# charlie-foxtrot/RTLSDR-Airband

Measured on AMD Instinct MI355X. Metric: IQ Msamples/sec channelized+demodulated per node; % HBM roofline, higher is better.
Workload: dtype i8x3->i32->f32 (stage 1), f32 (stage 2)

## Files before the change

### include/airband_hip.h

```cpp
#ifndef AIRBAND_HIP_H
#define AIRBAND_HIP_H

#include <stddef.h>
#include <stdint.h>

#ifdef __cplusplus
extern "C" {
#endif

#define AIRBAND_HIP_ABI_VERSION 2u

#define AIRBAND_HIP_OK 0
#define AIRBAND_HIP_ENODEV (-1)
#define AIRBAND_HIP_EBADSIZE (-2)
#define AIRBAND_HIP_ENOMEM (-3)
#define AIRBAND_HIP_EINVAL (-4)
#define AIRBAND_HIP_EAGAIN (-5)
#define AIRBAND_HIP_ERUNTIME (-6)

#define AIRBAND_SFMT_U8 1
#define AIRBAND_SFMT_S8 2
#define AIRBAND_SFMT_S16 3
#define AIRBAND_SFMT_F32 4

// ... 160 lines not shown
int airband_hip_collect_active(airband_hip_handle* h, int64_t* n_active, int32_t* channel_index, float* waveout, float* iq_out, char* axc_all);

int airband_hip_device_active(airband_hip_handle* h, int32_t** d_index, int32_t** d_count, float** d_rows, float** d_iq_rows);

int airband_hip_stream_wait_results(airband_hip_handle* h, void* stream);

int airband_hip_flush(airband_hip_handle* h);

int airband_hip_synchronize(airband_hip_handle* h);


int airband_hip_process_bins(airband_hip_handle* h, const float* wavein, const float* iq_in);

int airband_hip_read_bins(airband_hip_handle* h, float* wavein, float* iq_in);
int airband_hip_read_bins_channels(airband_hip_handle* h, int64_t first_channel, int64_t n_channels, float* wavein, float* iq_in);

int airband_hip_read_trace(airband_hip_handle* h, uint8_t* state);
int airband_hip_read_trace_channels(airband_hip_handle* h, int64_t first_channel, int64_t n_channels, uint8_t* state);

int airband_hip_channel_constants(const airband_hip_handle* h, int32_t channel_index, double* out_vals);

int airband_hip_derive_constants(const airband_hip_config* cfg, int32_t channel_index, double* out_vals);

int airband_hip_dft_selftest(const airband_hip_config* cfg, int32_t windows, double* max_rel_err);

int airband_hip_last_timings(airband_hip_handle* h, float* ms4);

int airband_hip_timing_totals(airband_hip_handle* h, double* ms4_sum, int64_t* n_batches, int32_t reset);

const char* airband_hip_build_info(void);

int airband_hip_regrouped(const airband_hip_handle* h);

const char* airband_hip_channelizer_name(const airband_hip_handle* h);

const char* airband_hip_channelizer_reason(const airband_hip_handle* h);

int64_t airband_hip_wide_hop_lds_bytes(int32_t fft_size, int32_t hop_bytes, int32_t sample_format);

int airband_hip_set_signal_plan(airband_hip_handle* h, const int64_t* carriers, int32_t n_carriers, int32_t noise_q8, const int16_t* sin_table4096);

int airband_hip_set_signal_plan_shift(airband_hip_handle* h, int32_t n_plans, uint32_t shift_step);

int airband_hip_generate_iq(airband_hip_handle* h, void* d_iq, size_t stride_bytes, uint64_t start_byte, size_t nbytes, uint64_t seed,
                            int32_t device_index_offset, void* stream);

#ifdef __cplusplus
}
#endif
#endif
```

### rtlsdr-airband_amd/__init__.py

```python
from __future__ import annotations

import ctypes as C
import importlib
import os
from typing import Optional, Sequence

import numpy as np

capi = importlib.import_module(__name__ + ".capi")
siggen = importlib.import_module(__name__ + ".siggen")
_build = importlib.import_module(__name__ + "._build")

HERE = os.path.dirname(os.path.abspath(__file__))
LIB_PATH = os.environ.get("AIRBAND_HIP_LIB") or os.path.join(HERE, "libairband_hip.so")

EXPORTS = [
    "airband_hip_prepare", "airband_hip_set_mixers", "airband_hip_release", "airband_hip_get_geometry", "airband_hip_last_error", "airband_hip_submit",
    "airband_hip_process", "airband_hip_process_device", "airband_hip_collect", "airband_hip_collect_mixers", "airband_hip_device_results",
    "airband_hip_synchronize", "airband_hip_process_bins", "airband_hip_read_bins", "airband_hip_read_trace", "airband_hip_channel_constants",
    "airband_hip_derive_constants", "airband_hip_last_timings", "airband_hip_channelizer_name", "airband_hip_set_signal_plan", "airband_hip_generate_iq",
    "airband_hip_flush", "airband_hip_timing_totals", "airband_hip_stream_wait_results", "airband_hip_mixer_enable_input",
    "airband_hip_device_enable", "airband_hip_gpu_count", "airband_hip_build_info", "airband_hip_dft_selftest", "airband_hip_collect_channels", "airband_hip_read_bins_channels", "airband_hip_read_trace_channels",
    "airband_hip_batch_ready", "airband_hip_mixer_set_stereo", "airband_hip_comm_unique_id", "airband_hip_comm_init_rank", "airband_hip_comm_init_all",
    "airband_hip_comm_group_begin", "airband_hip_comm_group_end", "airband_hip_allreduce_mixers", "airband_hip_add_mixers", "airband_hip_comm_destroy", "airband_hip_clear_mixers", "airband_hip_set_signal_plan_shift", "airband_hip_regrouped",
    "airband_hip_prepare_scan", "airband_hip_set_freq_index", "airband_hip_freq_stats",
    "airband_hip_set_output_gate", "airband_hip_collect_active", "airband_hip_device_active",
    "airband_hip_channelizer_reason", "airband_hip_wide_hop_lds_bytes",
]

_lib = None


class DevicePtr:

    def __init__(self, ptr: int, shape, typestr: str):
        self.__cuda_array_interface__ = dict(shape=tuple(shape), typestr=typestr, data=(int(ptr), False), version=2)


class AirbandError(RuntimeError):
    def __init__(self, code: int, text: str):
        super().__init__("airband_hip error %d: %s" % (code, text))
        self.code = code


def load_library() -> C.CDLL:
    global _lib
    if _lib is not None:
        return _lib
    if not os.path.exists(LIB_PATH):
        raise RuntimeError("libairband_hip.so is missing: run __graft_entry__.build() / python rtlsdr-airband_amd/_build.py (no CPU fallback exists)")
    try:
        import torch
    except Exception:
        pass
    L = C.CDLL(LIB_PATH)
    vp, i32, i64, u64, sz = C.c_void_p, C.c_int32, C.c_int64, C.c_uint64, C.c_size_t
    L.airband_hip_prepare.argtypes = [C.POINTER(capi.Config), C.POINTER(vp)]
    L.airband_hip_prepare_scan.argtypes = [C.POINTER(capi.Config), C.POINTER(capi.ScanCfg), i32, C.POINTER(vp)]
    L.airband_hip_set_freq_index.argtypes = [vp, i32, i32]
    L.airband_hip_freq_stats.argtypes = [vp, i32, i32, C.POINTER(capi.ChannelStats)]
# ... 14 lines not shown
    L.airband_hip_allreduce_mixers.argtypes = [vp, vp]
    L.airband_hip_add_mixers.argtypes = [vp, vp]
    L.airband_hip_comm_destroy.argtypes = [vp]
    L.airband_hip_clear_mixers.argtypes = [vp]
    L.airband_hip_comm_group_begin.argtypes = []
    L.airband_hip_comm_group_end.argtypes = []
    L.airband_hip_process_device.argtypes = [vp, vp, sz, vp]
    L.airband_hip_collect.argtypes = [vp, vp, vp, vp, vp]
    L.airband_hip_collect_channels.argtypes = [vp, i64, i64, vp, vp, vp, vp]
    L.airband_hip_read_bins_channels.argtypes = [vp, i64, i64, vp, vp]
    L.airband_hip_read_trace_channels.argtypes = [vp, i64, i64, vp]
    L.airband_hip_set_output_gate.argtypes = [vp, vp, i64]
    L.airband_hip_collect_active.argtypes = [vp, C.POINTER(i64), vp, vp, vp, vp]
    L.airband_hip_device_active.argtypes = [vp] + [C.POINTER(vp)] * 4
    L.airband_hip_collect_mixers.argtypes = [vp, vp, vp, vp]
    L.airband_hip_device_results.argtypes = [vp] + [C.POINTER(vp)] * 6
    L.airband_hip_synchronize.argtypes = [vp]
    L.airband_hip_process_bins.argtypes = [vp, vp, vp]
    L.airband_hip_read_bins.argtypes = [vp, vp, vp]
    L.airband_hip_read_trace.argtypes = [vp, vp]
    L.airband_hip_channel_constants.argtypes = [vp, i32, C.POINTER(C.c_double)]
    L.airband_hip_derive_constants.argtypes = [C.POINTER(capi.Config), i32, C.POINTER(C.c_double)]
    L.airband_hip_last_timings.argtypes = [vp, C.POINTER(C.c_float)]
    L.airband_hip_channelizer_name.argtypes = [vp]
    L.airband_hip_channelizer_name.restype = C.c_char_p
    L.airband_hip_channelizer_reason.argtypes = [vp]
    L.airband_hip_channelizer_reason.restype = C.c_char_p
    L.airband_hip_wide_hop_lds_bytes.argtypes = [i32, i32, i32]
    L.airband_hip_wide_hop_lds_bytes.restype = i64
    L.airband_hip_set_signal_plan.argtypes = [vp, vp, i32, i32, vp]
    L.airband_hip_generate_iq.argtypes = [vp, vp, sz, u64, sz, u64, i32, vp]
    L.airband_hip_set_signal_plan_shift.argtypes = [vp, i32, C.c_uint32]
    L.airband_hip_regrouped.argtypes = [vp]
    L.airband_hip_dft_selftest.argtypes = [C.POINTER(capi.Config), i32, C.POINTER(C.c_double)]
    L.airband_hip_build_info.argtypes = []
    L.airband_hip_build_info.restype = C.c_char_p
    L.airband_hip_flush.argtypes = [vp]
    L.airband_hip_mixer_enable_input.argtypes = [vp, i32, i32]
    L.airband_hip_device_enable.argtypes = [vp, i32, i32]
    L.airband_hip_gpu_count.argtypes = []
    L.airband_hip_stream_wait_results.argtypes = [vp, vp]
    L.airband_hip_timing_totals.argtypes = [vp, C.POINTER(C.c_double), C.POINTER(C.c_int64), i32]
    _lib = L
    return L


def make_config(devices: Sequence[dict], *, wave_rate: int, fft_log: int = 9, fm_demod: int = 0, flags: int = 0, hip_device: int = 0):
    keep, devs = [], []
    for dev in devices:
        dc, arr = capi.device_cfg(**dev)
        keep.append(arr)
        devs.append(dc)
    darr = (capi.DeviceCfg * len(devs))(*devs)
    keep.append(darr)
    cfg = capi.Config(capi.ABI_VERSION, flags, fft_log, wave_rate, fm_demod, hip_device, len(devs), C.cast(darr, C.POINTER(capi.DeviceCfg)))
    return cfg, keep


def derive_constants(devices: Sequence[dict], channel_index: int, *, wave_rate: int, fft_log: int = 9, fm_demod: int = 0):
    L = load_library()
    cfg, keep = make_config(devices, wave_rate=wave_rate, fft_log=fft_log, fm_demod=fm_demod)
    v = (C.c_double * 16)()
    rc = L.airband_hip_derive_constants(C.byref(cfg), channel_index, v)
    if rc != 0:
        raise AirbandError(rc, (L.airband_hip_last_error(None) or b"").decode())
    return list(v)
# ... 173 lines not shown
        w = np.empty((n, B), np.float32)
        q = np.empty((n, 2 * B), np.float32)
        self._check(self.L.airband_hip_read_bins_channels(self.h, int(first_channel), n, w.ctypes.data, q.ctypes.data))
        return w, q

    def read_trace(self, first_channel: int = 0, n_channels: Optional[int] = None) -> np.ndarray:
        n = self.total_channels - first_channel if n_channels is None else int(n_channels)
        t = np.empty((n, self.B), np.uint8)
        self._check(self.L.airband_hip_read_trace_channels(self.h, int(first_channel), n, t.ctypes.data))
        return t

    def constants(self, channel_index: int):
        v = (C.c_double * 16)()
        self._check(self.L.airband_hip_channel_constants(self.h, channel_index, v))
        return list(v)

    def last_timings(self):
        v = (C.c_float * 4)()
        self._check(self.L.airband_hip_last_timings(self.h, v))
        return dict(channelizer_ms=v[0], demod_ms=v[1], emit_ms=v[2], batch_ms=v[3])

    def timing_totals(self, reset: bool = False):
        v = (C.c_double * 4)()
        n = C.c_int64(0)
        self._check(self.L.airband_hip_timing_totals(self.h, v, C.byref(n), 1 if reset else 0))
        return dict(channelizer_ms=v[0], demod_ms=v[1], emit_ms=v[2], batch_ms=v[3], batches=int(n.value))

    def channelizer_name(self) -> str:
        return self.L.airband_hip_channelizer_name(self.h).decode()

    def channelizer_reason(self) -> str:
        return (self.L.airband_hip_channelizer_reason(self.h) or b"").decode()

    def build_info(self) -> str:
        return self.L.airband_hip_build_info().decode()

    def set_mixers(self, n_mixers: int, inputs: Sequence[tuple]):
        arr = (capi.MixerInput * len(inputs))(*[capi.MixerInput(int(a), int(b), int(c), float(d), float(e)) for a, b, c, d, e in inputs])
        self._check(self.L.airband_hip_set_mixers(self.h, n_mixers, arr, len(inputs)))
        self.n_mixers = n_mixers

    def mixer_enable_input(self, input_index: int, enabled: bool):
        self._check(self.L.airband_hip_mixer_enable_input(self.h, input_index, 1 if enabled else 0))

    def mixer_set_stereo(self, mixer: int, stereo: bool):
        self._check(self.L.airband_hip_mixer_set_stereo(self.h, int(mixer), 1 if stereo else 0))

    @staticmethod
    def comm_unique_id() -> bytes:
        buf = (C.c_uint8 * 128)()
        rc = load_library().airband_hip_comm_unique_id(buf)
        if rc < 0:
            raise AirbandError(rc, (load_library().airband_hip_last_error(None) or b"").decode())
        return bytes(buf)

    def comm_init_rank(self, unique_id: bytes, nranks: int, rank: int):
        assert len(unique_id) == 128
        self._check(self.L.airband_hip_comm_init_rank(self.h, (C.c_uint8 * 128).from_buffer_copy(unique_id), int(nranks), int(rank)))

    def allreduce_mixers(self, stream: int = 0):
        self._check(self.L.airband_hip_allreduce_mixers(self.h, C.c_void_p(stream)))

    def add_mixers(self, src: "AirbandHip"):
        self._check(self.L.airband_hip_add_mixers(self.h, src.h))

    def clear_mixers(self):
# ... 63 lines not shown
```

### rtlsdr-airband_amd/csrc/airband_hip.cpp

```cpp
#include <hip/hip_runtime.h>
#include <dlfcn.h>

#include <atomic>
#include <cstdio>
#include <cstdlib>
#include <cstring>
#include <memory>
#include <mutex>
#include <string>
#include <vector>

#include "handle.h"
#include "kernels.h"
#include "scan_bank.h"

#ifndef AB_PRIVATE_TABLE_BUDGET
#define AB_PRIVATE_TABLE_BUDGET ((size_t)8 << 30)
#endif

#ifndef AB_F32_TABLE_BUDGET
#define AB_F32_TABLE_BUDGET ((size_t)512 << 20)
#endif

using namespace airband;
// ... 79 lines not shown
        h->evp_state[i] = 0;
    }
    h->evp_state[i] |= (uint8_t)(1u << half);
    return h->evp[i];
}

void launch_retune_tables(airband_hip_handle* h, hipStream_t s, int epoch) {
    RetuneArgs ra;
    ra.cc = h->d_cc.p;
    ra.cs = h->d_cs.p;
    ra.dev = h->d_dev.p;
    ra.ext_to_slot = h->d_ext_to_slot.p;
    ra.item_dev = h->d_item_dev.p;
    ra.item_group = h->d_item_group.p;
    ra.item_bset = h->d_item_bset.p;
    ra.item_private = h->d_item_private.p;
    ra.item_home = h->d_item_home.p;
    ra.bset_bin = h->d_bset_bin.p;
    ra.bfrag = h->d_bfrag.p;
    ra.corr = h->d_bcorr.p;
    ra.ftab = h->use_f32 ? h->d_ftab.p : nullptr;
    ra.window = h->d_window.p;
    ra.n_items = (int)h->plan.item_dev.size();
    ra.fft_size = h->plan.fft_size;
    ra.n_shared = h->plan.n_shared_bsets;
    ra.moved_epoch = h->d_bset_bin.p + (size_t)h->plan.n_bsets * 8;
    ra.epoch = epoch;
    launch_retune(ra, s);
}

struct FrontRows {
    int first_row, n_hops;
};

FrontRows front_rows(const airband_hip_handle* h) {
    const bool first = h->front_batches == 0;
    return {first ? 0 : AB_AGC_EXTRA, first ? h->B + AB_AGC_EXTRA : h->B};
}

template <class Args>
void fill_front_args(Args& a, const airband_hip_handle* h, const void* d_iq, size_t stride_bytes, int row0, FrontRows r) {
    a.iq = (const uint8_t*)d_iq;
    a.iq_stride = (long)stride_bytes;
    a.dev = h->d_dev.p;
    a.cc = h->d_cc.p;
    a.ext_to_slot = h->d_ext_to_slot.p;
    a.mag = h->d_mag.p;
    a.iq_bins = h->d_iq.p;
    a.row0 = row0;
    a.ring_rows = h->R;
    a.first_row = r.first_row;
    a.n_hops = r.n_hops;
}

ChannelizerArgs fft_args(const airband_hip_handle* h, const void* d_iq, size_t stride_bytes, int row0, FrontRows r, int spectrum_only) {
    const Plan& p = h->plan;
    ChannelizerArgs ca;
    fill_front_args(ca, h, d_iq, stride_bytes, row0, r);
    ca.cs = h->d_cs.p;
    ca.window = h->d_window.p;
    ca.window_dec = h->d_window_dec.p;
    ca.twiddle = reinterpret_cast<const float2*>(h->d_twiddle.p);
    ca.last_spectrum = h->d_spectrum.p;
    ca.n_dev = p.n_dev;
    ca.fft_log = p.fft_log;
    ca.hop_samples = p.dev[0].hop_samples;
// ... 28 lines not shown
    a.splits = splits;
    return a;
}

DftArgs dft_args(const airband_hip_handle* h, const void* d_iq, size_t stride_bytes, FrontRows r) {
    const Plan& p = h->plan;
    DftArgs a;
    fill_front_args(a, h, d_iq, stride_bytes, h->row0_front, r);
    a.item_dev = h->d_item_dev.p;
    a.item_group = h->d_item_group.p;
    a.item_bset = h->d_item_bset.p;
    a.bfrag = h->d_bfrag.p;
    a.corr = h->d_bcorr.p;
    a.unscale = p.dev[0].sfmt == AIRBAND_SFMT_S16 ? p.b_unscale * 127.5 : p.dev[0].sfmt == AIRBAND_SFMT_S8 ? p.b_unscale * 127.5 / 128.0 : p.b_unscale;
    a.sfmt = p.dev[0].sfmt;
    a.edge_hi_zero = p.b_edge_hi_zero ? 1 : 0;
    a.n_dev = p.n_dev;
    a.n_items = (int)p.item_dev.size();
    a.fft_size = p.fft_size;
    a.hop_bytes = (int)h->hop_bytes;
    const int np_total = p.fft_size > 512 ? p.fft_size / 512 : 1, np = np_total > 8 ? 8 : np_total;
    const int win_bytes = 2 * p.fft_size * p.dev[0].bytes_per_sample / np_total * np;
    a.partial = reinterpret_cast<float4*>(h->d_dft_partial.p);
    if (h->use_wide) {
        a.lds_per_buf = dft_wide_lds_per_buf(win_bytes);
        a.nbuf = 2;
        a.sub = 1;
    } else {
        a.lds_per_buf = dft_lds_per_buf((int)h->hop_bytes, win_bytes, np);
        a.nbuf = dft_nbuf((int)h->hop_bytes, win_bytes, np);
        a.sub = dft_sub((int)h->hop_bytes, win_bytes, np);
    }
    a.extra_lds = 0;
    if (h->pipeline && np_total == 1) {
        const int used = a.nbuf * a.lds_per_buf, want = 28 * 1024;
        if (used < want) a.extra_lds = want - used;
    }
    const int steps = ((a.n_hops + 15) / 16 + 1 + a.sub - 1) / a.sub;
    int splits = (8192 + a.n_items - 1) / a.n_items;
    if (splits > steps / 4) splits = steps / 4;
    if (splits < 1) splits = 1;
    a.splits = splits;
    return a;
}

int launch_last_hop_spectrum(airband_hip_handle* h, hipStream_t s) {
    for (auto& e : h->ev_spec) HIP_TRY(h, e.ensure(), AIRBAND_HIP_ENODEV);
    (void)hipEventRecord(h->ev_spec[0], s);
    (void)hipStreamWaitEvent(h->side[0], h->ev_spec[0], 0);
    const uint8_t* last_hop = (const uint8_t*)h->last_iq + (size_t)(h->last_n_hops - 1) * (size_t)h->hop_bytes;
    launch_channelizer_fft(fft_args(h, last_hop, h->last_iq_stride, 0, FrontRows{0, 1}, 1), h->side[0]);
    (void)hipEventRecord(h->ev_spec[1], h->side[0]);
    return AIRBAND_HIP_OK;
}

ScanExchangeArgs scan_args(airband_hip_handle* h) {
    ScanExchangeArgs a;
    a.cc = h->d_cc.p;
    a.cs = h->d_cs.p;
    a.sqbuf = h->d_sqbuf.p;
    a.bank_cc = h->d_bank_cc.p;
    a.bank_cs = h->d_bank_cs.p;
    a.bank_sq = h->d_bank_sq.p;
    a.cs_mask = h->d_scan_mask.p;
    a.cc_mask = h->d_scan_mask.p + AB_CS_DWORDS;
    a.sw = nullptr;
    a.n_switch = 0;
// ... 136 lines not shown
    da.sq_key = h->d_sq_key.p;
    da.perm = (h->regroup && h->regroup_mode == 3) ? h->d_perm.p : nullptr;
    if (!h->plan.scan.empty()) {
        const int rc = scan_before_demod(h, s);
        if (rc != AIRBAND_HIP_OK) return rc;
    }
    hipStream_t side[3] = {h->side[0], h->side[1], h->side[2]};
    hipEvent_t fork_ev[4] = {h->fork_ev[0], h->fork_ev[1], h->fork_ev[2], h->fork_ev[3]};
    launch_demod(da, h->kind_first_block, h->kind_n_blocks, s, (h->flags & AIRBAND_HIP_FLAG_SERIAL_DEMOD) ? nullptr : side, fork_ev);
    if (h->any_afc && h->afc_spectrum_valid) {
        const bool tables = h->use_dft || h->use_f32;
        if (tables) (void)hipStreamWaitEvent(s, h->ev_spec[1], 0);
        const int epoch = (int)(h->batches_done % 0x7fffffff) + 1;
        launch_afc(h->d_cc.p, h->d_cs.p, h->d_spectrum.p, h->N, h->n_slots, tables ? h->d_bset_bin.p + (size_t)h->plan.n_bsets * 8 : nullptr, epoch, s);
        if (tables) launch_retune_tables(h, s, epoch);
        launch_axc(h->d_cc.p, h->d_cs.p, h->d_slot_to_ext.p, h->d_out_axc.p, h->n_slots, s);
    }
    (void)hipEventRecord(ev[3], s);
    if (h->d_out_iq.p) {
        EmitArgs ea;
        ea.iq_out = h->d_iq_out.p;
        ea.slot_to_ext = h->d_slot_to_ext.p;
        ea.out_iq = h->d_out_iq.p;
        ea.n_slots = h->n_slots;
        ea.wave_batch = h->B;
        launch_emit_iq(ea, s);
    }
    if (h->mix.n_mixers > 0) launch_mix(mix_args(h), s);
    if (h->gate.max_rows > 0) launch_gate(gate_args(h), s);
    (void)hipEventRecord(ev[4], s);
    hipError_t e = hipGetLastError();
    if (e != hipSuccess) return fail(h, AIRBAND_HIP_ERUNTIME, std::string("kernel launch: ") + hipGetErrorString(e));
    h->row0 = (h->row0 + h->B) % h->R;
    h->batches_done++;
    if (h->results_ready) h->overruns++;
    h->results_ready = true;
    harvest_timings(h, false);
    return AIRBAND_HIP_OK;
}

hipError_t write_mix_input(airband_hip_handle* h, int k) {
    const int ch = h->mix.chan_host[k];
    const int v = (h->mix.user_on[k] && h->dev_enabled[h->plan.cc[ch].dev]) ? ch : -1;
    hipError_t e = hipMemcpyAsync(h->mix.d_chan.p + k, &v, sizeof(int), hipMemcpyHostToDevice, h->stream);
    if (e != hipSuccess) return e;
    return hipStreamSynchronize(h->stream);
}


int prep_streams(airband_hip_handle* h) {
    HIP_TRY(PREPARING, hipSetDevice(h->hip_device), AIRBAND_HIP_ENODEV);
    int prio_lo = 0, prio_hi = 0;
    (void)hipDeviceGetStreamPriorityRange(&prio_lo, &prio_hi);
    HIP_TRY(PREPARING, hipStreamCreateWithPriority(&h->stream.v, hipStreamNonBlocking, prio_hi), AIRBAND_HIP_ENODEV);
    for (auto& set : h->evp)
        for (auto& e : set) HIP_TRY(PREPARING, hipEventCreate(&e.v), AIRBAND_HIP_ENODEV);
    if (h->pipeline) {
        HIP_TRY(PREPARING, hipStreamCreateWithFlags(&h->front.v, hipStreamNonBlocking), AIRBAND_HIP_ENODEV);
        HIP_TRY(PREPARING, h->ev_in.ensure(), AIRBAND_HIP_ENODEV);
        HIP_TRY(PREPARING, h->ev_back.ensure(), AIRBAND_HIP_ENODEV);
        for (auto& e : h->front_done) HIP_TRY(PREPARING, e.ensure(), AIRBAND_HIP_ENODEV);
    }
    for (auto& e : h->fork_ev) HIP_TRY(PREPARING, e.ensure(), AIRBAND_HIP_ENODEV);
    for (auto& st : h->side) HIP_TRY(PREPARING, hipStreamCreateWithPriority(&st.v, hipStreamNonBlocking, prio_lo), AIRBAND_HIP_ENODEV);
    return AIRBAND_HIP_OK;
}

int kind_of(const ChanConst& c) {
    if (c.flags & AB_F_IQ_OUT) return AB_KIND_GENERIC;
    const bool nfm = c.flags & AB_F_NFM, raw = c.flags & AB_F_RAW_IQ, lp = c.flags & AB_F_LOWPASS, ct = c.flags & AB_F_CTCSS;
    if (!nfm) return (!raw && !ct) ? AB_KIND_AM : AB_KIND_GENERIC;
    if (ct && lp) return AB_KIND_GENERIC;
    return ct ? AB_KIND_NFM_CTCSS : lp ? AB_KIND_NFM_LOWPASS : AB_KIND_NFM;
}

std::vector<int> channel_kinds(const Plan& p) {
    std::vector<int> kind_ext(p.total_ch);
    for (int e = 0; e < p.total_ch; e++) kind_ext[e] = kind_of(p.cc[e]);
    for (const ScanList& sl : p.scan) {
        int k = kind_of(p.scan_cc[sl.first_entry]);
        for (int f = 1; f < sl.n; f++)
            if (kind_of(p.scan_cc[sl.first_entry + f]) != k) k = AB_KIND_GENERIC;
        if (k == AB_KIND_NFM_LOWPASS && sl.n > 1) k = AB_KIND_GENERIC;
        kind_ext[sl.ext] = k;
    }
    return kind_ext;
}

void prep_slots(airband_hip_handle* h, std::vector<ChanState>& cs_slots, std::vector<uint8_t>& block_kind) {
    const Plan& p = h->plan;
    std::vector<ChanConst>& cc_slots = h->cc_slots;
    h->ext_to_slot.assign(p.total_ch, -1);
    const std::vector<int> kind_ext = channel_kinds(p);
    std::vector<uint8_t> isolated(p.total_ch, 0);
// ... 6 lines not shown
    pad_c.ct_slot = -1;
    pad_s.axc = ' ';
    auto pad_block = [&]() {
        while (cc_slots.size() % AB_SLOT_BLOCK) {
            h->slot_to_ext.push_back(-1);
            cc_slots.push_back(pad_c);
            cs_slots.push_back(pad_s);
        }
    };
    for (int k = 0; k < AB_KIND_COUNT; k++) {
        bool any = false;
        for (int pass = 0; pass < 2; pass++)
            for (int e = 0; e < p.total_ch; e++) {
                if (kind_ext[e] != k || isolated[e] != pass) continue;
                any = true;
                if (pass) pad_block();
                h->ext_to_slot[e] = (int)cc_slots.size();
                h->slot_to_ext.push_back(e);
                cc_slots.push_back(p.cc[e]);
                cs_slots.push_back(p.cs0[e]);
            }
        if (!any) continue;
        pad_block();
        h->kind_first_block[k] = (int)block_kind.size();
        while (block_kind.size() < cc_slots.size() / AB_SLOT_BLOCK) block_kind.push_back((uint8_t)k);
        h->kind_n_blocks[k] = (int)block_kind.size() - h->kind_first_block[k];
    }
    h->n_slots = (int)cc_slots.size();
}

void prep_geometry(airband_hip_handle* h) {
    const Plan& p = h->plan;
    h->B = p.wave_batch;
    h->R = ((h->pipeline ? 2 : 1) * p.wave_batch + AB_AGC_EXTRA + 15) / 16 * 16;
    h->N = p.fft_size;
    h->hop_bytes = 2LL * p.dev[0].bytes_per_sample * p.dev[0].hop_samples;
    h->first_batch_bytes = h->hop_bytes * (h->B + AB_AGC_EXTRA);
    h->batch_bytes = h->hop_bytes * h->B;
    h->lookahead_bytes = 2LL * p.dev[0].bytes_per_sample * p.fft_size - h->hop_bytes;
    if (h->lookahead_bytes < 0) h->lookahead_bytes = 0;
    h->lookahead_bytes += (16 - (h->batch_bytes + h->lookahead_bytes) % 16) % 16;
}

int prep_constants(airband_hip_handle* h, const std::vector<ChanState>& cs_slots, const std::vector<uint8_t>& block_kind) {
    const Plan& p = h->plan;
    HIP_TRY(PREPARING, upload(h->d_dev, p.dev), AIRBAND_HIP_ENOMEM);
    HIP_TRY(PREPARING, upload(h->d_cc, h->cc_slots), AIRBAND_HIP_ENOMEM);
    HIP_TRY(PREPARING, upload(h->d_cs, cs_slots), AIRBAND_HIP_ENOMEM);
    HIP_TRY(PREPARING, upload(h->d_slot_to_ext, h->slot_to_ext), AIRBAND_HIP_ENOMEM);
    HIP_TRY(PREPARING, upload(h->d_ext_to_slot, h->ext_to_slot), AIRBAND_HIP_ENOMEM);
    HIP_TRY(PREPARING, upload(h->d_block_kind, block_kind), AIRBAND_HIP_ENOMEM);
    HIP_TRY(PREPARING, upload(h->d_window, p.window), AIRBAND_HIP_ENOMEM);
    if (p.fft_size >= 1024) {
        const int M = p.fft_size / 512;
        std::vector<float> dec((size_t)p.fft_size);
        for (int n = 0; n < p.fft_size; n++) dec[(size_t)(n % M) * 512 + n / M] = p.window[n];
        HIP_TRY(PREPARING, upload(h->d_window_dec, dec), AIRBAND_HIP_ENOMEM);
    }
    HIP_TRY(PREPARING, upload(h->d_sin, p.sin_lut), AIRBAND_HIP_ENOMEM);
    HIP_TRY(PREPARING, upload(h->d_twiddle, p.twiddle), AIRBAND_HIP_ENOMEM);
    HIP_TRY(PREPARING, upload(h->d_cos, p.cos_lut), AIRBAND_HIP_ENOMEM);
    const int n_ct = (int)p.tones.size();
    h->ct_stride = n_ct;
    std::vector<float> coeff((size_t)(n_ct > 0 ? n_ct : 1) * 2 * AB_MAX_TONES, 0.0f);
    for (int s = 0; s < n_ct; s++)
        for (int k = 0; k < 2; k++)
            for (int t = 0; t < p.tones[s].n[k]; t++) coeff[((size_t)s * 2 + k) * AB_MAX_TONES + t] = p.tones[s].coeff[k][t];
// ... 235 lines not shown
        *max_rel_err = f32_table_selftest(plan, windows < 1 ? 1 : windows);
        return AIRBAND_HIP_OK;
    }
    const int wide_lds = (cfg->flags & AIRBAND_HIP_FLAG_WIDE_HOPS) ? dft_wide_lds(plan.fft_size, hop_bytes, plan.dev[0].sfmt) : -1;
    const bool wide = wide_lds >= 0 && wide_lds <= AB_DFT_WIDE_LDS_MAX;
    if (!plan.uniform_hop || !(wide || dft_supported(plan.fft_size, hop_bytes, plan.dev[0].sfmt, plan.max_ch)))
        return fail(nullptr, AIRBAND_HIP_EBADSIZE, "configuration does not take the matrix-core channelizer");
    build_dft_tables(plan);
    *max_rel_err = dft_table_selftest(plan, windows < 1 ? 1 : windows);
    return AIRBAND_HIP_OK;
}

int airband_hip_prepare(const airband_hip_config* cfg, airband_hip_handle** out) { return airband_hip_prepare_scan(cfg, nullptr, 0, out); }

int airband_hip_prepare_scan(const airband_hip_config* cfg, const airband_hip_scan_cfg* scan, int32_t n_scan, airband_hip_handle** out) {
    if (!out) return fail(nullptr, AIRBAND_HIP_EINVAL, "out is NULL");
    *out = nullptr;
    HandlePtr owner(new (std::nothrow) airband_hip_handle(), destroy);
    airband_hip_handle* const h = owner.get();
    if (!h) return fail(nullptr, AIRBAND_HIP_ENOMEM, "host allocation failed");
    int rc = build_plan(cfg, h->plan);
    if (rc == AIRBAND_HIP_OK) rc = build_scan(cfg, scan, n_scan, h->plan);
    if (rc != AIRBAND_HIP_OK) return fail(PREPARING, rc, h->plan.error);
    const Plan& p = h->plan;
    if (!p.uniform_hop)
        return fail(PREPARING, AIRBAND_HIP_EINVAL, "all dongles of one handle must share sample format and sample_rate/WAVE_RATE hop; use one handle per class");
    for (const ChanConst& c : p.cc) h->any_afc |= c.afc != 0;
    h->flags = cfg->flags;
    h->hip_device = cfg->hip_device;
    int ndev = 0;
    if (hipGetDeviceCount(&ndev) != hipSuccess || ndev <= 0 || cfg->hip_device < 0 || cfg->hip_device >= ndev)
        return fail(PREPARING, AIRBAND_HIP_ENODEV, "no usable HIP device (libairband_hip has no CPU fallback)");
    h->pipeline = (cfg->flags & AIRBAND_HIP_FLAG_PIPELINE) && !h->any_afc;
    rc = prep_streams(h);
    if (rc != AIRBAND_HIP_OK) return rc;
    std::vector<ChanState> cs_slots;
    std::vector<uint8_t> block_kind;
    prep_slots(h, cs_slots, block_kind);
    prep_geometry(h);
    rc = prep_constants(h, cs_slots, block_kind);
    if (rc == AIRBAND_HIP_OK) rc = prep_rings(h);
    if (rc == AIRBAND_HIP_OK) rc = prep_regroup(h);
    if (rc == AIRBAND_HIP_OK) rc = prep_results(h);
    if (rc == AIRBAND_HIP_OK) rc = prep_channelizer(h);
    if (rc != AIRBAND_HIP_OK) return rc;
    h->ring_wr.reset(new std::atomic<uint64_t>[p.n_dev]);
    for (int d = 0; d < p.n_dev; d++) h->ring_wr[d].store(0);
    h->dev_enabled.reset(new std::atomic<uint8_t>[p.n_dev]);
    for (int d = 0; d < p.n_dev; d++) h->dev_enabled[d].store(1);
    h->n_enabled = p.n_dev;
    if (!p.scan.empty()) rc = prep_scan(h);
    if (rc != AIRBAND_HIP_OK) return rc;
    *out = owner.release();
    return AIRBAND_HIP_OK;
}

void airband_hip_release(airband_hip_handle* h) { destroy(h); }

int airband_hip_get_geometry(const airband_hip_handle* h, airband_hip_geometry* g) {
    if (!h || !g) return AIRBAND_HIP_EINVAL;
    g->fft_size = h->N;
    g->wave_rate = h->plan.wave_rate;
    g->wave_batch = h->B;
    g->device_count = h->plan.n_dev;
    g->total_channels = h->plan.total_ch;
    g->max_channels = h->plan.max_ch;
// ... 157 lines not shown

int airband_hip_gpu_count(void) {
    int n = 0;
    if (hipGetDeviceCount(&n) != hipSuccess) return 0;
    return n;
}

static int launch_front(airband_hip_handle* h, const void* d_iq, size_t stride_bytes, hipStream_t s) {
    const FrontRows r = front_rows(h);
    const Event* ev = event_set(h, h->front_batches, 0);
    (void)hipGetLastError();
    h->afc_spectrum_valid = h->any_afc;
    if (h->use_f32 || h->use_dft) {
        h->last_iq = d_iq;
        h->last_iq_stride = stride_bytes;
        h->last_n_hops = r.n_hops;
        if (h->any_afc) {
            const int rc = launch_last_hop_spectrum(h, s);
            if (rc != AIRBAND_HIP_OK) return rc;
        }
    }
    (void)hipEventRecord(ev[0], s);
    if (h->use_f32) launch_channelizer_f32(f32_args(h, d_iq, stride_bytes, r), s);
    else if (h->use_wide) launch_channelizer_dft_wide(dft_args(h, d_iq, stride_bytes, r), s);
    else if (h->use_dft) launch_channelizer_dft(dft_args(h, d_iq, stride_bytes, r), s);
    else launch_channelizer_fft(fft_args(h, d_iq, stride_bytes, h->row0_front, r, 0), s);
    const hipError_t launch_err = hipGetLastError();
    (void)hipEventRecord(ev[1], s);
    if (launch_err != hipSuccess) return fail(h, AIRBAND_HIP_ERUNTIME, std::string("channelizer launch: ") + hipGetErrorString(launch_err));
    front_enqueued(h, r.first_row, r.n_hops);
    return AIRBAND_HIP_OK;
}

int airband_hip_process_device(airband_hip_handle* h, const void* d_iq, size_t stride_bytes, void* stream) {
    if (!h || !d_iq) return fail(h, AIRBAND_HIP_EINVAL, "NULL argument");
    HIP_TRY(h, hipSetDevice(h->hip_device), AIRBAND_HIP_ENODEV);
    uintptr_t al = 16;
    while (al > 2 && (h->hop_bytes % (int64_t)al) != 0) al >>= 1;
    if (al < (uintptr_t)(2 * h->plan.dev[0].bytes_per_sample)) al = (uintptr_t)(2 * h->plan.dev[0].bytes_per_sample);
    const uintptr_t need = al - 1;
    if (h->use_f32 && ((((uintptr_t)d_iq) | (uintptr_t)stride_bytes) & 15))
        return fail(h, AIRBAND_HIP_EINVAL, "d_iq and stride_bytes must be multiples of 16 (the channelizer fetches 16 bytes per lane)");
    if (h->use_dft && ((((uintptr_t)d_iq) | (uintptr_t)stride_bytes) & need))
        return fail(h, AIRBAND_HIP_EINVAL, (h->hop_bytes % 16) == 0 ? "d_iq and stride_bytes must be multiples of 16 (the channelizer fetches 16 bytes per lane)"
                                                                    : "d_iq and stride_bytes must be multiples of the largest power of two (up to 16) that divides the hop's bytes");
    if (!h->pipeline) {
        hipStream_t s = stream ? (hipStream_t)stream : h->stream;
        h->last_stream = s;
        const int rc_front = launch_front(h, d_iq, stride_bytes, s);
        if (rc_front != AIRBAND_HIP_OK) return rc_front;
        const int rc = run_back_half(h, s);
        if (s == h->stream) h->ev_last_pending = false;
        const int rc_mark = results_enqueued_on(h, s);
        return rc_mark != AIRBAND_HIP_OK ? rc_mark : rc;
    }
    hipStream_t in = stream ? (hipStream_t)stream : h->stream;
    HIP_TRY(h, hipEventRecord(h->ev_in, in), AIRBAND_HIP_ERUNTIME);
    HIP_TRY(h, hipStreamWaitEvent(h->front, h->ev_in, 0), AIRBAND_HIP_ERUNTIME);
    if (in != h->stream) {
        HIP_TRY(h, hipStreamWaitEvent(h->stream, h->ev_in, 0), AIRBAND_HIP_ERUNTIME);
        HIP_TRY(h, hipEventRecord(h->ev_back, h->stream), AIRBAND_HIP_ERUNTIME);
        HIP_TRY(h, hipStreamWaitEvent(h->front, h->ev_back, 0), AIRBAND_HIP_ERUNTIME);
    }
    const uint64_t k = h->front_batches;
    const int rc_front = launch_front(h, d_iq, stride_bytes, h->front);
    if (rc_front != AIRBAND_HIP_OK) return rc_front;
    HIP_TRY(h, hipEventRecord(h->front_done[k & 1], h->front), AIRBAND_HIP_ERUNTIME);
    if (h->batches_done == k) return AIRBAND_HIP_OK;
    HIP_TRY(h, hipStreamWaitEvent(h->stream, h->front_done[(k - 1) & 1], 0), AIRBAND_HIP_ERUNTIME);
    return run_back_half(h, h->stream);
}

int airband_hip_stream_wait_results(airband_hip_handle* h, void* stream) {
    if (!h || !stream) return fail(h, AIRBAND_HIP_EINVAL, "NULL argument");
    HIP_TRY(h, hipSetDevice(h->hip_device), AIRBAND_HIP_ENODEV);
    HIP_TRY(h, h->ev_wait.ensure(), AIRBAND_HIP_ENODEV);
    hipStream_t res = results_stream(h);
    if (res == (hipStream_t)stream) return AIRBAND_HIP_OK;
    HIP_TRY(h, hipEventRecord(h->ev_wait, res), AIRBAND_HIP_ERUNTIME);
    HIP_TRY(h, hipStreamWaitEvent((hipStream_t)stream, h->ev_wait, 0), AIRBAND_HIP_ERUNTIME);
    return AIRBAND_HIP_OK;
}

int airband_hip_flush(airband_hip_handle* h) {
    if (!h) return AIRBAND_HIP_EINVAL;
    if (!h->pipeline || h->front_batches == h->batches_done) return AIRBAND_HIP_OK;
    HIP_TRY(h, hipSetDevice(h->hip_device), AIRBAND_HIP_ENODEV);
    HIP_TRY(h, hipStreamWaitEvent(h->stream, h->front_done[(h->front_batches - 1) & 1], 0), AIRBAND_HIP_ERUNTIME);
    return run_back_half(h, h->stream);
}

static int64_t next_batch_bytes(const airband_hip_handle* h) { return h->front_batches == 0 ? h->first_batch_bytes : h->batch_bytes; }

static bool batch_available(const airband_hip_handle* h) {
    if (h->n_enabled == 0) return false;
    const int64_t need = next_batch_bytes(h) + h->lookahead_bytes;
    for (int d = 0; d < h->plan.n_dev; d++)
        if (h->dev_enabled[d] && (int64_t)(h->ring_wr[d].load(std::memory_order_acquire) - h->ring_rd) < need) return false;
    return true;
}

static int host_path_init(airband_hip_handle* h) {
    std::lock_guard<std::mutex> guard(h->host_init_lock);
    if (h->h_ring.load(std::memory_order_acquire)) return AIRBAND_HIP_OK;
// ... 39 lines not shown
    return batch_available(h) ? AIRBAND_HIP_OK : AIRBAND_HIP_EAGAIN;
}

int airband_hip_process(airband_hip_handle* h) {
    if (!h) return AIRBAND_HIP_EINVAL;
    HIP_TRY(h, hipSetDevice(h->hip_device), AIRBAND_HIP_ENODEV);
    if (!h->h_ring.load(std::memory_order_acquire)) {
        const int rc = host_path_init(h);
        if (rc != AIRBAND_HIP_OK) return rc;
    }
    uint8_t* const ring = h->h_ring.load(std::memory_order_acquire);
    if (!batch_available(h)) return AIRBAND_HIP_EAGAIN;
    const int64_t consume = next_batch_bytes(h);
    const int64_t need = consume + h->lookahead_bytes;
    const int b = (int)(h->host_batches & 1);
    if (h->host_batches > 0) {
        HIP_TRY(h, hipEventSynchronize(h->ev_h2d[b ^ 1]), AIRBAND_HIP_ERUNTIME);
        h->ring_free.store(h->ring_rd, std::memory_order_release);
    }
    if (h->host_batches >= 2) HIP_TRY(h, hipStreamWaitEvent(h->h2d, h->ev_stage_read[b], 0), AIRBAND_HIP_ERUNTIME);
    const size_t pos = (size_t)(h->ring_rd % (uint64_t)h->ring_cap);
    const size_t run = (size_t)need < (size_t)h->ring_cap - pos ? (size_t)need : (size_t)h->ring_cap - pos;
    HIP_TRY(h, hipMemcpy2DAsync(h->d_stage2[b].p, (size_t)h->stage_stride, ring + pos, (size_t)h->ring_cap, run, (size_t)h->plan.n_dev, hipMemcpyHostToDevice, h->h2d),
            AIRBAND_HIP_ERUNTIME);
    if (run < (size_t)need)
        HIP_TRY(h, hipMemcpy2DAsync(h->d_stage2[b].p + run, (size_t)h->stage_stride, ring, (size_t)h->ring_cap, (size_t)need - run, (size_t)h->plan.n_dev,
                                    hipMemcpyHostToDevice, h->h2d),
                AIRBAND_HIP_ERUNTIME);
    HIP_TRY(h, hipEventRecord(h->ev_h2d[b], h->h2d), AIRBAND_HIP_ERUNTIME);
    HIP_TRY(h, hipStreamWaitEvent(h->stream, h->ev_h2d[b], 0), AIRBAND_HIP_ERUNTIME);
    if (h->pipeline) HIP_TRY(h, hipStreamWaitEvent(h->front, h->ev_h2d[b], 0), AIRBAND_HIP_ERUNTIME);
    h->ring_rd += (uint64_t)consume;
    h->host_batches++;
    const int rc = airband_hip_process_device(h, h->d_stage2[b].p, (size_t)h->stage_stride, nullptr);
    (void)hipEventRecord(h->ev_stage_read[b], h->pipeline ? h->front : h->stream);
    return rc;
}

int airband_hip_process_bins(airband_hip_handle* h, const float* wavein, const float* iq_in) {
    if (!h || !wavein || !iq_in) return fail(h, AIRBAND_HIP_EINVAL, "NULL argument");
    if (h->pipeline) return fail(h, AIRBAND_HIP_EINVAL, "process_bins (stage 2 only) is not available on a pipelined handle");
    HIP_TRY(h, hipSetDevice(h->hip_device), AIRBAND_HIP_ENODEV);
    const size_t n = (size_t)h->plan.total_ch * h->B;
    HIP_TRY(h, h->d_tmp_wavein.reserve(n), AIRBAND_HIP_ENOMEM);
    HIP_TRY(h, h->d_tmp_iqin.reserve(2 * n), AIRBAND_HIP_ENOMEM);
    hipStream_t s = h->stream;
    HIP_TRY(h, hipMemcpyAsync(h->d_tmp_wavein.p, wavein, n * sizeof(float), hipMemcpyHostToDevice, s), AIRBAND_HIP_ERUNTIME);
    HIP_TRY(h, hipMemcpyAsync(h->d_tmp_iqin.p, iq_in, 2 * n * sizeof(float), hipMemcpyHostToDevice, s), AIRBAND_HIP_ERUNTIME);
    const Event* ev = event_set(h, h->front_batches, 0);
    (void)hipEventRecord(ev[0], s);
    h->afc_spectrum_valid = false;
    launch_scatter_bins(h->d_tmp_wavein.p, h->d_tmp_iqin.p, h->d_slot_to_ext.p, h->d_cc.p, h->d_mag.p, h->d_iq.p, h->n_slots, h->B, h->row0, h->R, s);
    (void)hipEventRecord(ev[1], s);
    front_enqueued(h, AB_AGC_EXTRA, h->B);
    return run_back_half(h, s);
}

int airband_hip_synchronize(airband_hip_handle* h) {
    if (!h) return AIRBAND_HIP_EINVAL;
    HIP_TRY(h, hipSetDevice(h->hip_device), AIRBAND_HIP_ENODEV);
    if (h->front) HIP_TRY(h, hipStreamSynchronize(h->front), AIRBAND_HIP_ERUNTIME);
    if (h->ev_last && h->ev_last_pending) HIP_TRY(h, hipEventSynchronize(h->ev_last), AIRBAND_HIP_ERUNTIME);
    HIP_TRY(h, hipStreamSynchronize(h->stream), AIRBAND_HIP_ERUNTIME);
    return AIRBAND_HIP_OK;
}

static int collect_range(airband_hip_handle* h, int64_t first, int64_t n, float* waveout, float* iq_out, char* axc, airband_hip_channel_stats* stats, bool consume) {
    if (!h) return AIRBAND_HIP_EINVAL;
    if (first < 0 || n < 0 || first + n > h->plan.total_ch) return fail(h, AIRBAND_HIP_EINVAL, "channel range out of bounds");
    if (!h->results_ready && consume) return AIRBAND_HIP_EAGAIN;
    if (h->batches_done == 0) return AIRBAND_HIP_EAGAIN;
    HIP_TRY(h, hipSetDevice(h->hip_device), AIRBAND_HIP_ENODEV);
    hipStream_t s = h->stream;
    order_behind_last_batch(h);
    const size_t nch = (size_t)n;
    if (stats && nch) {
        if (!h->d_stats.p) HIP_TRY(h, h->d_stats.alloc((size_t)h->plan.total_ch), AIRBAND_HIP_ENOMEM);
        launch_stats(h->d_cc.p, h->d_cs.p, h->d_slot_to_ext.p, h->n_slots, h->d_stats.p, s);
        HIP_TRY(h, hipMemcpyAsync(stats, h->d_stats.p + first, nch * sizeof(airband_hip_channel_stats), hipMemcpyDeviceToHost, s), AIRBAND_HIP_ERUNTIME);
// ... 171 lines not shown
    return AIRBAND_HIP_OK;
}

int airband_hip_last_timings(airband_hip_handle* h, float* ms4) {
    if (!h || !ms4) return AIRBAND_HIP_EINVAL;
    HIP_TRY(h, hipSetDevice(h->hip_device), AIRBAND_HIP_ENODEV);
    harvest_timings(h, true);
    if (!h->timings_valid) return AIRBAND_HIP_EAGAIN;
    for (int k = 0; k < 4; k++) ms4[k] = h->t_last[k];
    return AIRBAND_HIP_OK;
}

int airband_hip_timing_totals(airband_hip_handle* h, double* ms4_sum, int64_t* n_batches, int32_t reset) {
    if (!h) return AIRBAND_HIP_EINVAL;
    HIP_TRY(h, hipSetDevice(h->hip_device), AIRBAND_HIP_ENODEV);
    harvest_timings(h, true);
    if (ms4_sum)
        for (int k = 0; k < 4; k++) ms4_sum[k] = h->t_sum[k];
    if (n_batches) *n_batches = h->t_n[0];
    if (reset) {
        for (double& v : h->t_sum) v = 0.0;
        h->t_n[0] = 0;
    }
    return AIRBAND_HIP_OK;
}

#ifndef AB_BUILD_DEFINES
#define AB_BUILD_DEFINES ""
#endif
const char* airband_hip_build_info(void) { return AB_BUILD_DEFINES; }

int airband_hip_regrouped(const airband_hip_handle* h) { return (h && h->regroup) ? 1 : 0; }

const char* airband_hip_channelizer_name(const airband_hip_handle* h) {
    return (h && h->use_dft) ? "dft_mfma_i8" : (h && h->use_f32) ? "dft_mfma_f32" : "fft_wave64";
}

const char* airband_hip_channelizer_reason(const airband_hip_handle* h) { return h ? h->chan_reason.c_str() : ""; }

int64_t airband_hip_wide_hop_lds_bytes(int32_t fft_size, int32_t hop_bytes, int32_t sample_format) { return dft_wide_lds(fft_size, hop_bytes, sample_format); }

int airband_hip_set_signal_plan(airband_hip_handle* h, const int64_t* carriers, int32_t n_carriers, int32_t noise_q8, const int16_t* sin_table4096) {
    if (!h || !carriers || !sin_table4096 || n_carriers < 1 || n_carriers > 16) return fail(h, AIRBAND_HIP_EINVAL, "bad signal plan (1..16 carriers)");
    HIP_TRY(h, hipSetDevice(h->hip_device), AIRBAND_HIP_ENODEV);
    std::vector<long long> c(carriers, carriers + (size_t)n_carriers * 12);
    std::vector<int16_t> t(sin_table4096, sin_table4096 + 4096);
    HIP_TRY(h, upload(h->d_carriers, c), AIRBAND_HIP_ENOMEM);
    HIP_TRY(h, upload(h->d_sin_tab, t), AIRBAND_HIP_ENOMEM);
    h->n_carriers = n_carriers;
    h->noise_q8 = noise_q8;
    return AIRBAND_HIP_OK;
}

int airband_hip_set_signal_plan_shift(airband_hip_handle* h, int32_t n_plans, uint32_t shift_step) {
    if (!h || n_plans < 1 || n_plans > 65536) return fail(h, AIRBAND_HIP_EINVAL, "bad plan count (1..65536)");
    h->sig_n_plans = n_plans;
    h->sig_shift_step = shift_step;
    return AIRBAND_HIP_OK;
}

int airband_hip_generate_iq(airband_hip_handle* h, void* d_iq, size_t stride_bytes, uint64_t start_byte, size_t nbytes, uint64_t seed, int32_t device_index_offset,
                            void* stream) {
    if (!h || !d_iq) return fail(h, AIRBAND_HIP_EINVAL, "NULL argument");
    if (h->n_carriers == 0) return fail(h, AIRBAND_HIP_EINVAL, "call airband_hip_set_signal_plan first");
    if (h->plan.dev[0].sfmt != AIRBAND_SFMT_U8) return fail(h, AIRBAND_HIP_EINVAL, "the synthetic generator emits u8 I/Q");
    if ((start_byte & 1) || (nbytes & 1)) return fail(h, AIRBAND_HIP_EINVAL, "byte ranges must cover whole I/Q pairs");
    HIP_TRY(h, hipSetDevice(h->hip_device), AIRBAND_HIP_ENODEV);
    SiggenArgs a;
    a.iq = (uint8_t*)d_iq;
    a.stride = (long)stride_bytes;
    a.sin_tab = h->d_sin_tab.p;
    a.carriers = h->d_carriers.p;
    a.n_carriers = h->n_carriers;
    a.n_dev = h->plan.n_dev;
    a.dev_offset = device_index_offset;
    a.start_sample = start_byte / 2;
    a.n_samples = (long)(nbytes / 2);
    a.seed = seed;
    a.noise_q8 = h->noise_q8;
    a.n_plans = h->sig_n_plans;
    a.plan_shift_step = h->sig_shift_step;
    launch_siggen(a, stream ? (hipStream_t)stream : h->stream);
    hipError_t e = hipGetLastError();
    if (e != hipSuccess) return fail(h, AIRBAND_HIP_ERUNTIME, std::string("siggen launch: ") + hipGetErrorString(e));
    return AIRBAND_HIP_OK;
}

namespace {
struct Rccl {
    void* dl = nullptr;
    ncclResult_t (*GetUniqueId)(ncclUniqueId*) = nullptr;
    ncclResult_t (*CommInitRank)(ncclComm_t*, int, ncclUniqueId, int) = nullptr;
    ncclResult_t (*CommInitAll)(ncclComm_t*, int, const int*) = nullptr;
    ncclResult_t (*AllReduce)(const void*, void*, size_t, ncclDataType_t, ncclRedOp_t, ncclComm_t, hipStream_t) = nullptr;
    ncclResult_t (*CommDestroy)(ncclComm_t) = nullptr;
    ncclResult_t (*GroupStart)() = nullptr;
    ncclResult_t (*GroupEnd)() = nullptr;
    const char* (*GetErrorString)(ncclResult_t) = nullptr;
    bool named = false;
    bool shared_gpu_ok = false;
    std::string why;
};
Rccl g_rccl;
std::mutex g_rccl_lock;

Rccl* rccl() {
    std::lock_guard<std::mutex> guard(g_rccl_lock);
    if (g_rccl.dl) return &g_rccl;
    if (!g_rccl.why.empty()) return nullptr;
    void* dl = nullptr;
    std::string tried;
    const char* named = getenv("AIRBAND_HIP_RCCL_LIB");
    if (named && *named) {
        dl = dlopen(named, RTLD_NOW | RTLD_GLOBAL);
        if (!dl) {
// ... 176 lines not shown
```

### rtlsdr-airband_amd/csrc/handle.h

```cpp
#pragma once

#include <hip/hip_runtime.h>
#include <rccl/rccl.h>

#include <atomic>
#include <memory>
#include <mutex>
#include <string>
#include <utility>
#include <vector>

#include "../../include/airband_hip.h"
#include "common.h"
#include "params.h"

namespace airband {

template <class H, hipError_t (*Release)(H)>
struct Owned {
    H v = nullptr;
    Owned() = default;
    Owned(Owned&& o) noexcept : v(std::exchange(o.v, nullptr)) {}
    Owned& operator=(Owned&& o) noexcept {
        std::swap(v, o.v);
// ... 49 lines not shown

struct MixerWiring {
    std::vector<int> pos;
    std::vector<int> chan_host;
    std::vector<uint8_t> user_on;
    int n_mixers = 0;
    int n_runs = 0;
    DevBuf<int> d_chan, d_first, d_run_first, d_run_mixer, d_first_run;
    DevBuf<float> d_run_left, d_run_right;
    DevBuf<uint8_t> d_run_signal;
    DevBuf<float> d_ml, d_mr, d_left, d_right;
    DevBuf<uint8_t> d_stereo, d_signal;
};

struct OutputGate {
    int max_rows = 0;
    std::vector<uint8_t> gate;
    DevBuf<uint8_t> d_gate, d_prev;
    DevBuf<unsigned long long> d_mask;
    DevBuf<int> d_block_count, d_index, d_count;
    DevBuf<float> d_rows, d_iq_rows;
};

}

struct airband_hip_handle {
    airband::Plan plan;
    uint32_t flags = 0;
    int hip_device = 0;
    airband::Stream stream;
    airband::Stream side[3];
    airband::Event fork_ev[4];
    bool pipeline = false;
    airband::Stream front;
    airband::Event ev_in, ev_back, ev_wait, front_done[2];
    hipStream_t last_stream = nullptr;
    airband::Event ev_spec[2];
    airband::Event ev_last;
    bool ev_last_pending = false;
    int row0_front = 0;
    uint64_t front_batches = 0;
    static constexpr int EV_POOL = 16;
    airband::Event evp[EV_POOL][5];
    uint8_t evp_state[EV_POOL] = {0};
    double t_sum[4] = {0, 0, 0, 0};
    int64_t t_n[2] = {0, 0};
    float t_last[4] = {0, 0, 0, 0};
    bool timings_valid = false;
    std::string error;

    int B = 0, R = 0, N = 0;
    int n_slots = 0;
    std::vector<int> slot_to_ext, ext_to_slot;
    int kind_first_block[AB_KIND_COUNT] = {0}, kind_n_blocks[AB_KIND_COUNT] = {0};
    int64_t hop_bytes = 0, first_batch_bytes = 0, batch_bytes = 0, lookahead_bytes = 0;
    int row0 = 0;
    int wave_stride = 0;
    uint64_t batches_done = 0;
    bool results_ready = false;
    uint64_t overruns = 0;

    airband::DevBuf<DevConst> d_dev;
    airband::DevBuf<ChanConst> d_cc;
    airband::DevBuf<ChanState> d_cs;
    airband::DevBuf<int> d_slot_to_ext, d_ext_to_slot;
    airband::DevBuf<uint8_t> d_block_kind;
    airband::DevBuf<float> d_window, d_sin, d_cos, d_twiddle;
    airband::DevBuf<float> d_window_dec;
// ... 81 lines not shown
```

Baseline: 1.460 million.

## Run channelizer front half ahead on separate stream with double-buffered rings

Adds a default-on run-ahead mode for device-pointer submissions. The channelizer front stage runs on its own stream, so batch k+1's front can overlap batch k's back half, with back_done/front_done events guarding the two-deep ring. The ring depth doubles and the channelizer gets extra LDS padding to limit waves per CU, as in pipeline mode. Host-bin, siggen and host-ring paths set a flag that forces serialisation, which adds event and synchronisation complexity and the risk of ordering bugs.

New measurement: 1.555 million, median of 6. 1.07x the previous value.

```diff
diff --git a/include/airband_hip.h b/include/airband_hip.h
--- a/include/airband_hip.h
+++ b/include/airband_hip.h
@@ -216,6 +216,8 @@
 
 int airband_hip_regrouped(const airband_hip_handle* h);
 
+int airband_hip_schedule_info(const airband_hip_handle* h, int32_t* run_ahead, int32_t* ring_batches, int32_t* channelizer_waves_per_cu, int64_t* batches_run_ahead);
+
 const char* airband_hip_channelizer_name(const airband_hip_handle* h);
 
 const char* airband_hip_channelizer_reason(const airband_hip_handle* h);
diff --git a/rtlsdr-airband_amd/__init__.py b/rtlsdr-airband_amd/__init__.py
--- a/rtlsdr-airband_amd/__init__.py
+++ b/rtlsdr-airband_amd/__init__.py
@@ -25,7 +25,7 @@
     "airband_hip_comm_group_begin", "airband_hip_comm_group_end", "airband_hip_allreduce_mixers", "airband_hip_add_mixers", "airband_hip_comm_destroy", "airband_hip_clear_mixers", "airband_hip_set_signal_plan_shift", "airband_hip_regrouped",
     "airband_hip_prepare_scan", "airband_hip_set_freq_index", "airband_hip_freq_stats",
     "airband_hip_set_output_gate", "airband_hip_collect_active", "airband_hip_device_active",
-    "airband_hip_channelizer_reason", "airband_hip_wide_hop_lds_bytes",
+    "airband_hip_channelizer_reason", "airband_hip_wide_hop_lds_bytes", "airband_hip_schedule_info",
 ]
 
 _lib = None
@@ -106,6 +106,7 @@
     L.airband_hip_generate_iq.argtypes = [vp, vp, sz, u64, sz, u64, i32, vp]
     L.airband_hip_set_signal_plan_shift.argtypes = [vp, i32, C.c_uint32]
     L.airband_hip_regrouped.argtypes = [vp]
+    L.airband_hip_schedule_info.argtypes = [vp, C.POINTER(i32), C.POINTER(i32), C.POINTER(i32), C.POINTER(i64)]
     L.airband_hip_dft_selftest.argtypes = [C.POINTER(capi.Config), i32, C.POINTER(C.c_double)]
     L.airband_hip_build_info.argtypes = []
     L.airband_hip_build_info.restype = C.c_char_p
@@ -345,6 +346,11 @@
     def channelizer_reason(self) -> str:
         return (self.L.airband_hip_channelizer_reason(self.h) or b"").decode()
 
+    def schedule_info(self) -> dict:
+        a, b, c, n = C.c_int32(0), C.c_int32(0), C.c_int32(0), C.c_int64(0)
+        self._check(self.L.airband_hip_schedule_info(self.h, C.byref(a), C.byref(b), C.byref(c), C.byref(n)))
+        return dict(run_ahead=bool(a.value), ring_batches=int(b.value), channelizer_waves_per_cu=int(c.value), batches_run_ahead=int(n.value))
+
     def build_info(self) -> str:
         return self.L.airband_hip_build_info().decode()
 
diff --git a/rtlsdr-airband_amd/csrc/airband_hip.cpp b/rtlsdr-airband_amd/csrc/airband_hip.cpp
--- a/rtlsdr-airband_amd/csrc/airband_hip.cpp
+++ b/rtlsdr-airband_amd/csrc/airband_hip.cpp
@@ -135,6 +135,8 @@
 struct FrontRows {
     int first_row, n_hops;
 };
+
+bool deep_rings(const airband_hip_handle* h) { return h->pipeline || h->run_ahead; }
 
 FrontRows front_rows(const airband_hip_handle* h) {
     const bool first = h->front_batches == 0;
@@ -229,7 +231,7 @@
         a.sub = dft_sub((int)h->hop_bytes, win_bytes, np);
     }
     a.extra_lds = 0;
-    if (h->pipeline && np_total == 1) {
+    if (deep_rings(h) && np_total == 1) {
         const int used = a.nbuf * a.lds_per_buf, want = 28 * 1024;
         if (used < want) a.extra_lds = want - used;
     }
@@ -432,6 +434,7 @@
     hipError_t e = hipGetLastError();
     if (e != hipSuccess) return fail(h, AIRBAND_HIP_ERUNTIME, std::string("kernel launch: ") + hipGetErrorString(e));
     h->row0 = (h->row0 + h->B) % h->R;
+    if (h->run_ahead && s == h->stream) (void)hipEventRecord(h->back_done[h->batches_done & 1], s);
     h->batches_done++;
     if (h->results_ready) h->overruns++;
     h->results_ready = true;
@@ -455,11 +458,13 @@
     HIP_TRY(PREPARING, hipStreamCreateWithPriority(&h->stream.v, hipStreamNonBlocking, prio_hi), AIRBAND_HIP_ENODEV);
     for (auto& set : h->evp)
         for (auto& e : set) HIP_TRY(PREPARING, hipEventCreate(&e.v), AIRBAND_HIP_ENODEV);
-    if (h->pipeline) {
+    if (deep_rings(h)) {
         HIP_TRY(PREPARING, hipStreamCreateWithFlags(&h->front.v, hipStreamNonBlocking), AIRBAND_HIP_ENODEV);
         HIP_TRY(PREPARING, h->ev_in.ensure(), AIRBAND_HIP_ENODEV);
         HIP_TRY(PREPARING, h->ev_back.ensure(), AIRBAND_HIP_ENODEV);
         for (auto& e : h->front_done) HIP_TRY(PREPARING, e.ensure(), AIRBAND_HIP_ENODEV);
+        if (h->run_ahead)
+            for (auto& e : h->back_done) HIP_TRY(PREPARING, e.ensure(), AIRBAND_HIP_ENODEV);
     }
     for (auto& e : h->fork_ev) HIP_TRY(PREPARING, e.ensure(), AIRBAND_HIP_ENODEV);
     for (auto& st : h->side) HIP_TRY(PREPARING, hipStreamCreateWithPriority(&st.v, hipStreamNonBlocking, prio_lo), AIRBAND_HIP_ENODEV);
@@ -532,7 +537,7 @@
 void prep_geometry(airband_hip_handle* h) {
     const Plan& p = h->plan;
     h->B = p.wave_batch;
-    h->R = ((h->pipeline ? 2 : 1) * p.wave_batch + AB_AGC_EXTRA + 15) / 16 * 16;
+    h->R = ((deep_rings(h) ? 2 : 1) * p.wave_batch + AB_AGC_EXTRA + 15) / 16 * 16;
     h->N = p.fft_size;
     h->hop_bytes = 2LL * p.dev[0].bytes_per_sample * p.dev[0].hop_samples;
     h->first_batch_bytes = h->hop_bytes * (h->B + AB_AGC_EXTRA);
@@ -834,6 +839,8 @@
     if (hipGetDeviceCount(&ndev) != hipSuccess || ndev <= 0 || cfg->hip_device < 0 || cfg->hip_device >= ndev)
         return fail(PREPARING, AIRBAND_HIP_ENODEV, "no usable HIP device (libairband_hip has no CPU fallback)");
     h->pipeline = (cfg->flags & AIRBAND_HIP_FLAG_PIPELINE) && !h->any_afc;
+    const char* run_ahead_env = getenv("AIRBAND_HIP_RUN_AHEAD");
+    h->run_ahead = !(cfg->flags & AIRBAND_HIP_FLAG_PIPELINE) && !h->any_afc && p.scan.empty() && !(run_ahead_env && *run_ahead_env == '0');
     rc = prep_streams(h);
     if (rc != AIRBAND_HIP_OK) return rc;
     std::vector<ChanState> cs_slots;
@@ -1057,7 +1064,7 @@
     return AIRBAND_HIP_OK;
 }
 
-int airband_hip_process_device(airband_hip_handle* h, const void* d_iq, size_t stride_bytes, void* stream) {
+static int process_batch(airband_hip_handle* h, const void* d_iq, size_t stride_bytes, void* stream, bool run_ahead_ok) {
     if (!h || !d_iq) return fail(h, AIRBAND_HIP_EINVAL, "NULL argument");
     HIP_TRY(h, hipSetDevice(h->hip_device), AIRBAND_HIP_ENODEV);
     uintptr_t al = 16;
@@ -1069,9 +1076,30 @@
     if (h->use_dft && ((((uintptr_t)d_iq) | (uintptr_t)stride_bytes) & need))
         return fail(h, AIRBAND_HIP_EINVAL, (h->hop_bytes % 16) == 0 ? "d_iq and stride_bytes must be multiples of 16 (the channelizer fetches 16 bytes per lane)"
                                                                     : "d_iq and stride_bytes must be multiples of the largest power of two (up to 16) that divides the hop's bytes");
+    if (h->run_ahead && !stream && run_ahead_ok) {
+        const uint64_t k = h->front_batches;
+        if (h->ev_last_pending) order_behind_last_batch(h);
+        if (h->serialise_next) {
+            HIP_TRY(h, hipEventRecord(h->ev_in, h->stream), AIRBAND_HIP_ERUNTIME);
+            HIP_TRY(h, hipStreamWaitEvent(h->front, h->ev_in, 0), AIRBAND_HIP_ERUNTIME);
+        } else if (k >= 2) {
+            HIP_TRY(h, hipStreamWaitEvent(h->front, h->back_done[k & 1], 0), AIRBAND_HIP_ERUNTIME);
+        }
+        h->serialise_next = false;
+        h->last_stream = h->stream;
+        const int rc_front = launch_front(h, d_iq, stride_bytes, h->front);
+        if (rc_front != AIRBAND_HIP_OK) return rc_front;
+        HIP_TRY(h, hipEventRecord(h->front_done[k & 1], h->front), AIRBAND_HIP_ERUNTIME);
+        HIP_TRY(h, hipStreamWaitEvent(h->stream, h->front_done[k & 1], 0), AIRBAND_HIP_ERUNTIME);
+        const int rc = run_back_half(h, h->stream);
+        h->ev_last_pending = false;
+        h->ahead_batches++;
+        return rc;
+    }
     if (!h->pipeline) {
         hipStream_t s = stream ? (hipStream_t)stream : h->stream;
         h->last_stream = s;
+        if (h->run_ahead) h->serialise_next = true;
         const int rc_front = launch_front(h, d_iq, stride_bytes, s);
         if (rc_front != AIRBAND_HIP_OK) return rc_front;
         const int rc = run_back_half(h, s);
@@ -1095,6 +1123,8 @@
     HIP_TRY(h, hipStreamWaitEvent(h->stream, h->front_done[(k - 1) & 1], 0), AIRBAND_HIP_ERUNTIME);
     return run_back_half(h, h->stream);
 }
+
+int airband_hip_process_device(airband_hip_handle* h, const void* d_iq, size_t stride_bytes, void* stream) { return process_batch(h, d_iq, stride_bytes, stream, true); }
 
 int airband_hip_stream_wait_results(airband_hip_handle* h, void* stream) {
     if (!h || !stream) return fail(h, AIRBAND_HIP_EINVAL, "NULL argument");
@@ -1200,7 +1230,7 @@
     if (h->pipeline) HIP_TRY(h, hipStreamWaitEvent(h->front, h->ev_h2d[b], 0), AIRBAND_HIP_ERUNTIME);
     h->ring_rd += (uint64_t)consume;
     h->host_batches++;
-    const int rc = airband_hip_process_device(h, h->d_stage2[b].p, (size_t)h->stage_stride, nullptr);
+    const int rc = process_batch(h, h->d_stage2[b].p, (size_t)h->stage_stride, nullptr, false);
     (void)hipEventRecord(h->ev_stage_read[b], h->pipeline ? h->front : h->stream);
     return rc;
 }
@@ -1213,6 +1243,10 @@
     HIP_TRY(h, h->d_tmp_wavein.reserve(n), AIRBAND_HIP_ENOMEM);
     HIP_TRY(h, h->d_tmp_iqin.reserve(2 * n), AIRBAND_HIP_ENOMEM);
     hipStream_t s = h->stream;
+    if (h->run_ahead) {
+        if (h->ahead_batches > 0) HIP_TRY(h, hipStreamWaitEvent(s, h->front_done[(h->front_batches - 1) & 1], 0), AIRBAND_HIP_ERUNTIME);
+        h->serialise_next = true;
+    }
     HIP_TRY(h, hipMemcpyAsync(h->d_tmp_wavein.p, wavein, n * sizeof(float), hipMemcpyHostToDevice, s), AIRBAND_HIP_ERUNTIME);
     HIP_TRY(h, hipMemcpyAsync(h->d_tmp_iqin.p, iq_in, 2 * n * sizeof(float), hipMemcpyHostToDevice, s), AIRBAND_HIP_ERUNTIME);
     const Event* ev = event_set(h, h->front_batches, 0);
@@ -1450,6 +1484,16 @@
 
 int airband_hip_regrouped(const airband_hip_handle* h) { return (h && h->regroup) ? 1 : 0; }
 
+int airband_hip_schedule_info(const airband_hip_handle* h, int32_t* run_ahead, int32_t* ring_batches, int32_t* channelizer_waves_per_cu, int64_t* batches_run_ahead) {
+    if (!h) return AIRBAND_HIP_EINVAL;
+    if (run_ahead) *run_ahead = h->run_ahead ? 1 : 0;
+    if (ring_batches) *ring_batches = (h->R - AB_AGC_EXTRA) / h->B;
+    if (channelizer_waves_per_cu)
+        *channelizer_waves_per_cu = (h->use_dft && dft_args(h, nullptr, 0, FrontRows{AB_AGC_EXTRA, h->B}).extra_lds > 0) ? 5 : 0;
+    if (batches_run_ahead) *batches_run_ahead = (int64_t)h->ahead_batches;
+    return AIRBAND_HIP_OK;
+}
+
 const char* airband_hip_channelizer_name(const airband_hip_handle* h) {
     return (h && h->use_dft) ? "dft_mfma_i8" : (h && h->use_f32) ? "dft_mfma_f32" : "fft_wave64";
 }
@@ -1499,6 +1543,7 @@
     a.n_plans = h->sig_n_plans;
     a.plan_shift_step = h->sig_shift_step;
     launch_siggen(a, stream ? (hipStream_t)stream : h->stream);
+    if (!stream && h->run_ahead) h->serialise_next = true;
     hipError_t e = hipGetLastError();
     if (e != hipSuccess) return fail(h, AIRBAND_HIP_ERUNTIME, std::string("siggen launch: ") + hipGetErrorString(e));
     return AIRBAND_HIP_OK;
diff --git a/rtlsdr-airband_amd/csrc/handle.h b/rtlsdr-airband_amd/csrc/handle.h
--- a/rtlsdr-airband_amd/csrc/handle.h
+++ b/rtlsdr-airband_amd/csrc/handle.h
@@ -105,8 +105,12 @@
     airband::Stream side[3];
     airband::Event fork_ev[4];
     bool pipeline = false;
+    bool run_ahead = false;
+    bool serialise_next = false;
+    uint64_t ahead_batches = 0;
     airband::Stream front;
     airband::Event ev_in, ev_back, ev_wait, front_done[2];
+    airband::Event back_done[2];
     hipStream_t last_stream = nullptr;
     airband::Event ev_spec[2];
     airband::Event ev_last;
```
